# pavel-paulau/query

Hardware: AMD Instinct MI355X
Metric: rows/sec filter+group-by on 100M synthetic JSON docs; achieved HBM GB/s (higher is better)
Workload: dtype int64/f64 tagged scalars (u8 tag + 8 B payload), u32 dictionary codes; 1 GPU; config2: SELECT cat, SUM(price) FROM default WHERE price > 50 GROUP BY cat @ 100000000 rows, K_cat=1000, columns resident in HBM; rows_per_gpu=100000000, groups=1000, rows_selected=49401294, agg_mode=2, spec_kernel=1

## Files before the change

query_amd/build.py:

```python
from __future__ import annotations

import os
import shutil
import subprocess
import sys

HERE = os.path.dirname(os.path.abspath(__file__))
CSRC = os.path.join(HERE, "csrc")
LIB = os.path.join(HERE, "libn1k.so")
SOURCES = ["n1k_kernels.hip", "n1k_bins.hip", "n1k_jsondev.hip", "n1k_matchtable.hip", "n1k_order.hip", "n1k_rowdistinct.hip", "n1k_mathfn.hip", "n1k_arrfn.hip", "n1k_datefn.hip", "n1k_order.cpp", "n1k_rowdistinct.cpp", "n1k_matchtable.cpp", "n1k_like.cpp", "n1k_coll.cpp", "n1k_arrfn.cpp", "n1k_datefn.cpp", "n1k_in.cpp", "n1k_strfn.cpp", "n1k_jsonpush.cpp", "n1k_plan.cpp", "n1k_engine.cpp", "n1k_scan.cpp", "n1k_select.cpp", "n1k_partitioned.cpp", "n1k_distinct.cpp",
           "n1k_finish.cpp", "n1k_tail.cpp", "n1k_exchange.cpp", "n1k_jit.cpp", "n1k_json.cpp"]
HEADERS = ["n1k_types.h", "n1k_device.h", "n1k_tables.h", "n1k_fold.h", "n1k_scatter.h", "n1k_spec.h", "n1k_like.h", "n1k_coll.h", "n1k_arrfn.h", "n1k_datefn.h", "n1k_cond.h", "n1k_in.h", "n1k_strfn.h", "n1k_order.h", "n1k_rowdistinct.h", "n1k_jit.h", "n1k_kernels.h", "n1k_plan.h", os.path.join("..", "..", "include", "n1k.h")]
HOST_HEADERS = ["n1k_engine.h", "n1k_buf.h", "n1k_wire.h"]
ARCH = "gfx950"


def _hipcc() -> str:
    for c in (os.environ.get("HIPCC"), shutil.which("hipcc"), "/opt/rocm/bin/hipcc"):
        if c and os.path.exists(c):
            return c
    raise RuntimeError("hipcc not found")


OBJDIR = os.path.join(CSRC, "build")
FLAGS = ["--offload-arch=" + ARCH, "-O3", "-std=c++17", "-fPIC", "-munsafe-fp-atomics", "-Wall", "-Wno-unused-function"]


def _stale(target: str, deps) -> bool:
    if not os.path.exists(target):
        return True
    mt = os.path.getmtime(target)
    return any(os.path.getmtime(d) > mt for d in deps)


def source_hash() -> str:
    import hashlib
    h = hashlib.sha1()
    for f in sorted([x for x in SOURCES if x.endswith(".hip")] + [x for x in HEADERS if not x.startswith("..")]):
        with open(os.path.join(CSRC, f), "rb") as fh:
            h.update(f.encode() + b"\0" + fh.read())
    return h.hexdigest()[:16]


def needs_build() -> bool:
    return _stale(LIB, [os.path.join(CSRC, f) for f in SOURCES + HEADERS + HOST_HEADERS] + [os.path.abspath(__file__)])
# ... 33 lines not shown
```

query_amd/csrc/n1k_engine.h:

```cpp
#pragma once
#include <hip/hip_runtime.h>

#include <algorithm>
#include <atomic>
#include <chrono>
#include <cmath>
#include <cstdarg>
#include <cstdio>
#include <cstring>
#include <functional>
#include <numeric>
#include <string>
#include <condition_variable>
#include <mutex>
#include <thread>
#include <unordered_map>
#include <vector>

#include "../../include/n1k.h"
#include "n1k_buf.h"
#include "n1k_jit.h"
#include "n1k_json.h"
#include "n1k_kernels.h"
#include "n1k_arrfn.h"
// ... 148 lines not shown
    uint32_t jit = 1;
    uint64_t jit_min_rows = 4u << 20;
    uint32_t distinct_words = 1;
    uint32_t distinct_set_slots = 8192;
    uint32_t records = 1;
    uint32_t rec_slots = 0, rec_bins = 0, rec_slices = 0, rec_scan_per_cu = 0, rec_block = 0, rec_unroll = 0;
    uint64_t region_cap = 0;
    uint32_t dedupe_block = 1025;
    uint32_t json_device = 1;
    uint32_t json_device_left_pct = 12;
    uint64_t json_device_min_docs = 4096;
    uint32_t json_threads = 0;
    uint64_t partition_min_rows = 8u << 20, partition_probe_rows = 512u << 10, partition_min_groups = 4096;
    uint32_t partition_sticky = 1;
    int32_t partition_levels = -1;
    uint64_t topk_min_groups = 65536;
    int32_t distinct_levels = -1;
    uint64_t wide_values = 1u << 20;
    uint32_t slabs = 1;
    uint32_t block = 0, rows_per_lane = 4;
    uint32_t lds_bytes = 64 * 1024;
    uint32_t rep_row = 0;
    uint64_t rowdistinct_slots = 0;
    uint32_t rowdistinct_lds_slots = 0;
};

enum Counter : uint32_t {
    CTR_ROWS_SELECTED = 0,
    CTR_GROUPS = 1,
    CTR_OUT_COUNT = 2,
    CTR_FILTER_TOTAL = 3,
    CTR_REHASH_SCRATCH = 4,
    CTR_DISTINCT_REGION_WORDS = 5,
    CTR_TAIL_TICKET = 6,
    CTR_PAIR_LOG_CURSORS = 8,
    CTR_ERR_FLAGS = 12,
    CTR_WIDE_VALUES = 13,
    CTR_WORD_LOG_CURSORS = 16,
    CTR_OPTIMISTIC_OVERFLOW = 20,
    CTR_PART_RECORDS = 21,
    CTR_SINGLETONS = 22,
    CTR_EXACT_OVERFLOW = 24,
    CTR_SAVED_ROWS_SELECTED = 25,
    CTR_REGION_GROUPS = 26,
    CTR_PEER_STATUS = 27,
    CTR_ROWDISTINCT_COUNT = 28,
    CTR_ROWDISTINCT_REACHED = 29
};
static_assert(CTR_ERR_FLAGS + kPeerStatusFromErr == CTR_PEER_STATUS, "the verdict kernel writes the peer status this far behind the flags");
static_assert(CTR_ROWDISTINCT_REACHED < kCounters && CTR_ROWDISTINCT_REACHED == CTR_ROWDISTINCT_COUNT + 1, "every counter word lies inside the buffer (CTR_ROWDISTINCT_REACHED is the last)");
static_assert(CTR_ROWS_SELECTED == 0 && CTR_GROUPS == 1 && CTR_OUT_COUNT == 2 && CTR_TAIL_TICKET > CTR_DISTINCT_REGION_WORDS && CTR_TAIL_TICKET < CTR_PAIR_LOG_CURSORS,
              "the query's last kernels (finalize_small_kernel, fold_rows_kernel) write words [0], [1] and [2] by number");
static_assert(CTR_PAIR_LOG_CURSORS + kMaxDistinct <= CTR_ERR_FLAGS && CTR_WORD_LOG_CURSORS + kMaxDistinct <= CTR_OPTIMISTIC_OVERFLOW, "cursor words overlap their neighbours");

struct GroupTable {
    GlobalTable table{};
    DevBuf<uint64_t> keys, acc, rep;
    DevBuf<uint64_t> slabs;
    DevBuf<unsigned long long> block_sel;
    uint32_t* errp = nullptr;
    DevBuf<unsigned long long> counters;
    DevBuf<uint64_t> wide_int, wide_flt;
    uint64_t merged_bound = 0;
    struct PendingSlabs {
        bool clean_at_push = false;
        uint32_t grid = 0;
        FastArgs F{};
    } pending;
};
uint32_t intern(n1k_handle* h, const std::string& s);
uint32_t lookup_code(const n1k_handle* h, const char* s);
bool to_operand(n1k_handle* h, const Expr* e, Operand& o, PlanError& err);
bool compile_plan(n1k_handle* h, PlanError& err);
n1k_status ensure_device(n1k_handle* h);
n1k_status reset_handle(n1k_handle* h, bool clear_stop);
n1k_status ensure_rank(n1k_handle* h);
n1k_status fix_layout(n1k_handle* h, const n1k_batch* b);
n1k_status ensure_table(n1k_handle* h, uint64_t incoming_rows);
n1k_status ensure_table_groups(n1k_handle* h, uint64_t groups);
hipEvent_t get_event(n1k_handle* h);
n1k_status ensure_pinned_counters(n1k_handle* h);
void drain_events(n1k_handle* h);
n1k_status validate_batch(n1k_handle* h, const n1k_batch* b);
uint64_t batch_bytes_per_row(const n1k_handle* h);
void default_value(const AggDef& d, n1k_value& v, n1k_partial& p);
// ... 126 lines not shown
struct Distinct {
    DevBuf<uint64_t> log_key[kMaxDistinct], log_val[kMaxDistinct], regions, set_table;
    DevBuf<uint8_t> log_cls[kMaxDistinct];
    DevBuf<uint64_t> log_word[kMaxDistinct], part[2], seg[3], wtable;
    DevBuf<unsigned long long> hist, cursor, dcounts, word_hist;
    DevBuf<uint64_t> wregion[kMaxDistinct], woff, wgather;
    DevBuf<unsigned long long> wcursor;
    uint64_t wregion_cap = 0;
    bool wregion_used = false;
    uint32_t nw_key_bits = 0, nw_val_bits = 0;
    bool words[kMaxDistinct] = {false, false, false, false};
    uint32_t path = 0;
    uint64_t log_capacity = 0;
};
n1k_status distinct_grow_logs(n1k_handle* h, uint64_t nrows, ScanArgs& A);
n1k_status distinct_grow_regions(n1k_handle* h, const Program& P, uint64_t nrows, const ScanArgs& A, uint32_t dcache_slots, WordLogArgs& L);
n1k_status distinct_words_finish(n1k_handle* h, const AggSpec& ag, uint64_t nwords, bool hist_counted = true, const uint64_t* log = nullptr);
n1k_status distinct_regions_finish(n1k_handle* h, const AggSpec& ag, uint64_t nover, bool force_exact, bool* deferred);

struct TopK {
    DevBuf<uint64_t> images;
    DevBuf<uint32_t> cand;
    DevBuf<char> state, out2;
};
struct Results {
    std::vector<n1k_value> keys, aggs;
    std::vector<n1k_partial> parts;
    std::vector<uint64_t> rep;
    DevBuf<char> d_out;
    std::vector<char> out_host;
    std::vector<char> export_blob;
    bool out_count_dirty = true;
    PinBuf<char> pin_out;
    PinBuf<unsigned long long> pin_counters;
    PinBuf<char> pin_rows;
};

struct Tail {
    n1k_handle* project = nullptr;
    std::vector<int> project_cols;
    std::vector<Operand> project_ops;
    std::vector<n1k_value> r_proj;
    n1k_handle* having = nullptr;
    std::vector<int> having_cols;
    std::vector<uint32_t> having_codes;
};
n1k_status build_projection(n1k_handle* h);
n1k_status having_groups(n1k_handle* h, uint64_t& ng);
n1k_status project_groups(n1k_handle* h, uint64_t ng);
n1k_status order_groups(n1k_handle* h, uint64_t& ng);
n1k_status array_agg_groups(n1k_handle* h, uint64_t ng, const unsigned long long* counters);
bool slabs_to_rows(const n1k_handle* h, const FastArgs& F, uint32_t g, bool only_chunk, bool whole);
void publish_result(n1k_handle* h, uint64_t ng, bool partials, n1k_result* out);

}

using namespace n1k_eng;

struct n1k_handle {
    ParsedPlan plan;
    std::string last_error;
    std::atomic<int> stop_flag{0};
    Options opt;
    bool failure_global = false;
    bool device_clean = false, clear_on_finish = false;
    std::string jit_log;
// ... 74 lines not shown
```

query_amd/csrc/n1k_finish.cpp:

```cpp
#include "n1k_engine.h"

using namespace n1k;
using namespace n1k_eng;

static void mark_query_end(n1k_handle* h) {
    if (h->timing.q0_recorded && h->timing.ev_q1 && hipEventRecord(h->timing.ev_q1, h->stream) == hipSuccess) h->timing.q1_recorded = true;
}

struct OutLayout {
    size_t aggs, parts, rep, total;
    OutLayout(uint64_t groups = 0, size_t nk = 0, size_t na = 0)
        : aggs(groups * nk * sizeof(OutValue)), parts(aggs + groups * na * sizeof(OutValue)), rep(parts + groups * na * sizeof(OutPartial)), total(rep + groups * 8) {}
    OutValue* k(char* b) const { return (OutValue*)b; }
    OutValue* a(char* b) const { return (OutValue*)(b + aggs); }
    OutPartial* p(char* b) const { return (OutPartial*)(b + parts); }
    uint64_t* r(char* b) const { return (uint64_t*)(b + rep); }
};

struct Finish {
    unsigned long long counters[kCounters] = {0};
    uint32_t err_flags = 0;
    uint64_t ng = 0;
    uint64_t spec_groups = 0;
    char* d_rows = nullptr;
    char* rows = nullptr;
    OutLayout lay;
    bool sets_exact = false;
    bool sets_deferred = false, vetoed = false;
    std::chrono::steady_clock::time_point wait_end{};
};

enum : uint32_t { PIN_NCAND = kCounters, PIN_ERR_FLAGS, PIN_VETO };

static uint64_t speculative_groups(const n1k_handle* h) {
    const ParsedPlan& pl = h->plan;
    const bool topk_forced = pl.has_order && pl.limit >= 0 && !pl.has_having && h->opt.topk_min_groups < 4096;
    if (!pl.has_group || h->has_distinct || !h->groups.table.capacity || h->groups.table.capacity > (1u << 20) || topk_forced || h->part.pending.count)
        return 0;
    return std::min<uint64_t>(h->groups.table.capacity, 4096);
}

namespace n1k_eng {
bool slabs_to_rows(const n1k_handle* h, const FastArgs& F, uint32_t g, bool only_chunk, bool whole) {
    if (!h->clear_on_finish || !h->groups.pending.clean_at_push || !only_chunk || !whole || h->push_nrows_dev || h->push_nseg) return false;
    if (!F.slabs || F.hashed || g <= 1 || h->opt.merge_chunks != 0 || h->prog.wide_int || h->has_array_agg) return false;
    const uint64_t spec = speculative_groups(h), cap = h->groups.table.capacity;
    return spec && cap <= kFinalizeSmallMax && F.lds_slots <= std::min<uint64_t>(std::min<uint64_t>(cap, spec), h->opt.max_groups);
}
}

static n1k_status zero_out_count(n1k_handle* h) {
    if (h->res.out_count_dirty) HIP_TRY(h, hipMemsetAsync(h->groups.counters.p + CTR_OUT_COUNT, 0, sizeof(unsigned long long), h->stream));
    h->res.out_count_dirty = true;
    return N1K_OK;
}

static n1k_status read_counters(n1k_handle* h, Finish& F) {
    if (!h->device_ready) return h->timing.stats.rows_in == 0 ? ensure_device(h) : N1K_OK;
    HIP_TRY(h, hipSetDevice(h->device));
    ST_TRY(ensure_pinned_counters(h));
    GroupTable::PendingSlabs& ps = h->groups.pending;
    const bool fold = ps.grid && slabs_to_rows(h, ps.F, ps.grid, true, true);
    if (ps.grid && !fold) {
        HIP_TRY(h, launch_merge_slabs(h->prog, ps.F, h->groups.table, ps.grid, h->groups.counters.p + CTR_GROUPS, h->stream, h->opt.merge_chunks));
        ps.grid = 0;
    }
    F.spec_groups = speculative_groups(h);
    if (F.spec_groups) {
        F.lay = OutLayout(F.spec_groups, h->plan.keys.size(), h->plan.aggs.size());
        HIP_TRY(h, h->res.pin_out.ensure(F.lay.total + kCounters * sizeof(unsigned long long)));
        char* d = F.rows = h->res.pin_out.p;
        unsigned long long* host_counters = (unsigned long long*)(d + F.lay.total);
        if (fold) {
            HIP_TRY(h, launch_fold_rows(h->prog, ps.F, h->groups.table, ps.grid, F.lay.k(d), F.lay.a(d), F.lay.p(d), F.lay.r(d), h->groups.counters.p, CTR_TAIL_TICKET,
                                        host_counters, F.spec_groups, h->stream));
            ps.grid = 0;
            h->res.out_count_dirty = false;
            h->device_clean = true;
        } else if (h->groups.table.capacity <= kFinalizeSmallMax) {
            const bool clear = h->clear_on_finish && !h->prog.wide_int;
            HIP_TRY(h, launch_finalize_small(h->prog, h->groups.table, F.lay.k(d), F.lay.a(d), F.lay.p(d), F.lay.r(d), h->groups.counters.p,
                                             host_counters, F.spec_groups, h->groups.errp, clear, h->stream));
            h->res.out_count_dirty = !clear;
            h->device_clean = clear;
        } else {
            ST_TRY(zero_out_count(h));
            HIP_TRY(h, launch_finalize(h->prog, h->groups.table, F.lay.k(d), F.lay.a(d), F.lay.p(d), F.lay.r(d),
                                       h->groups.counters.p + CTR_OUT_COUNT, F.spec_groups, h->groups.errp, h->stream));
            HIP_TRY(h, launch_publish_counters(h->groups.counters.p, host_counters, kCounters, h->stream));
        }
        mark_query_end(h);
        const auto w0 = std::chrono::steady_clock::now();
        HIP_TRY(h, hipStreamSynchronize(h->stream));
        F.wait_end = std::chrono::steady_clock::now();
        h->timing.host_us[3] += std::chrono::duration<double, std::micro>(F.wait_end - w0).count();
        memcpy(F.counters, host_counters, sizeof F.counters);
        if (fold && F.counters[CTR_TAIL_TICKET]) {
            h->device_clean = false;
            F.counters[CTR_TAIL_TICKET] = 0;
        }
    } else {
        HIP_TRY(h, hipMemcpyAsync(h->res.pin_counters.p, h->groups.counters.p, sizeof F.counters, hipMemcpyDeviceToHost, h->stream));
        mark_query_end(h);
        HIP_TRY(h, hipStreamSynchronize(h->stream));
        memcpy(F.counters, h->res.pin_counters.p, sizeof F.counters);
    }
    F.err_flags = (uint32_t)F.counters[CTR_ERR_FLAGS];
    drain_events(h);
    return N1K_OK;
}

static n1k_status build_distinct_sets(n1k_handle* h, Finish& F) {
    h->distinct.path = 0;
    if (h->distinct.wregion_used) HIP_TRY(h, hipMemsetAsync(h->groups.counters.p + CTR_OPTIMISTIC_OVERFLOW, 0, 8, h->stream));
    for (size_t a = 0; a < h->plan.aggs.size(); a++) {
        const AggSpec& ag = h->prog.aggs[a];
        if (!ag.distinct || ag.kind == AGG_ARRAY) continue;
        const uint64_t npairs = std::min<uint64_t>(F.counters[CTR_PAIR_LOG_CURSORS + ag.log_index], h->distinct.log_capacity);
        const uint64_t nwords = h->distinct.words[ag.log_index] ? std::min<uint64_t>(F.counters[CTR_WORD_LOG_CURSORS + ag.log_index], h->distinct.log_capacity) : 0;
        DistinctArgs D{};
        D.log_key = h->distinct.log_key[ag.log_index].p;
        D.log_val = h->distinct.log_val[ag.log_index].p;
        D.log_cls = h->distinct.log_cls[ag.log_index].p;
        D.npairs = npairs;
        D.glob_off = ag.glob_off;
        D.kind = ag.kind;
        D.total_words = h->groups.counters.p + CTR_DISTINCT_REGION_WORDS;
        HIP_TRY(h, h->distinct.regions.ensure(h->groups.table.capacity * 6));
        D.regions = h->distinct.regions.p;
        HIP_TRY(h, hipMemsetAsync(D.total_words, 0, sizeof(unsigned long long), h->stream));
        HIP_TRY(h, launch_distinct_layout(h->prog, h->groups.table, D, h->stream));
        if (npairs) {
            unsigned long long words = 0;
// ... 70 lines not shown
    F.lay = OutLayout(ncand, nk, na);
    HIP_TRY(h, h->topk.out2.ensure(F.lay.total + 16));
    char* c = F.d_rows = h->topk.out2.p;
    if (tk.lean)
        HIP_TRY(h, launch_finalize_region(h->prog, h->part.emit.p, h->part.pending.cap, ncand, F.lay.k(c), F.lay.a(c), F.lay.p(c), F.lay.r(c),
                                          h->groups.errp, h->stream, h->topk.cand.p));
    else
        HIP_TRY(h, launch_topk_compact(h->topk.cand.p, ncand, nk, na, all.k(d), all.a(d), all.p(d), all.r(d), F.lay.k(c), F.lay.a(c), F.lay.p(c),
                                       F.lay.r(c), h->stream));
    h->timing.stats.topk_candidates = ncand;
    F.ng = ncand;
    return N1K_OK;
}

static n1k_status land_rows(n1k_handle* h, Finish& F) {
    const size_t bytes = F.lay.total;
    const bool pinned_rows = bytes <= (8u << 20);
    if (pinned_rows && h->res.pin_rows.n < bytes) HIP_TRY(h, h->res.pin_rows.ensure(std::max<size_t>(bytes, 64u << 10)));
    if (!pinned_rows) h->res.out_host.resize(bytes);
    F.rows = pinned_rows ? h->res.pin_rows.p : h->res.out_host.data();
    unsigned long long* const pin = h->res.pin_counters.p;
    HIP_TRY(h, hipMemcpyAsync(F.rows, F.d_rows, bytes, hipMemcpyDeviceToHost, h->stream));
    HIP_TRY(h, hipMemcpyAsync(pin + PIN_ERR_FLAGS, h->groups.errp, 4, hipMemcpyDeviceToHost, h->stream));
    if (F.sets_deferred) HIP_TRY(h, hipMemcpyAsync(pin + PIN_VETO, h->groups.counters.p + CTR_OPTIMISTIC_OVERFLOW, 8, hipMemcpyDeviceToHost, h->stream));
    mark_query_end(h);
    HIP_TRY(h, hipStreamSynchronize(h->stream));
    memcpy(&F.err_flags, pin + PIN_ERR_FLAGS, 4);
    F.vetoed = F.sets_deferred && pin[PIN_VETO] != 0;
    return N1K_OK;
}

static void unpack_rows(n1k_handle* h, const Finish& F) {
    const size_t nk = h->plan.keys.size(), na = h->plan.aggs.size(), ng = F.ng;
    h->res.keys.assign((const n1k_value*)F.lay.k(F.rows), (const n1k_value*)F.lay.k(F.rows) + ng * nk);
    h->res.aggs.assign((const n1k_value*)F.lay.a(F.rows), (const n1k_value*)F.lay.a(F.rows) + ng * na);
    h->res.rep.assign(F.lay.r(F.rows), F.lay.r(F.rows) + ng);
    const OutPartial* parts = F.lay.p(F.rows);
    h->res.parts.resize(ng * na);
    for (size_t i = 0; i < ng * na; i++) {
        n1k_partial& p = h->res.parts[i];
        memset(&p, 0, sizeof p);
        p.count = parts[i].count;
        p.isum = parts[i].isum;
        p.fsum = parts[i].fsum;
        p.int_exact = parts[i].flags & 1u;
        p.has_float = (parts[i].flags >> 1) & 1u;
        p.extreme.tag = (uint8_t)parts[i].ext_tag;
        p.extreme.v.code = parts[i].ext_payload;
        p.distinct = parts[i].distinct;
    }
}

static n1k_status flags_status(n1k_handle* h, const Finish& F) {
    if (F.err_flags & kErrFromVerdict) {
        h->failure_global = true;
        if (F.err_flags & ERR_PEER_FAILED) {
            const int ps = (int)(F.counters[CTR_PEER_STATUS] & 0xFF);
            return fail(h, ps > 0 && ps <= N1K_REGION_FULL ? (n1k_status)ps : N1K_DEVICE_ERROR,
                        "a rank failed before the exchange (its status: %d); the step is void on every rank", ps);
        }
        if (F.err_flags & ERR_EXCHANGE_WIDE)
            return fail(h, N1K_UNSUPPORTED, "a sender's group keys hold float / wide integer values: use the row exchange");
        if (F.err_flags & ERR_EXCHANGE_OVERFLOW)
            return fail(h, N1K_REGION_FULL, "a sender's region overflowed: raise the region capacity (on every rank)");
        if (F.err_flags & ERR_PEER_UNPACKABLE)
            return fail(h, N1K_UNSUPPORTED_DATA, "a sender met a group key value that does not fit the packed key (option wide_values, or a key layout too narrow)");
        return fail(h, N1K_UNSUPPORTED_DATA, "a sender met a value outside the device subset (ordering of arrays/objects)");
    }
    if (F.err_flags & ERR_TABLE_FULL)
        return fail(h, N1K_OOM, "group table capacity exceeded: raise the max_groups option (now %llu)",
                    (unsigned long long)h->opt.max_groups);
    if (F.err_flags & ERR_UNPACKABLE_KEY)
        return fail(h, N1K_UNSUPPORTED_DATA,
                    "a group key value does not fit the packed key: more than %llu distinct float / wide integer key "
                    "values (option wide_values), or a key layout too narrow for them",
                    (unsigned long long)((1ull << h->prog.wide_bits) / 2));
    if (F.err_flags & ERR_UNSUPPORTED_VALUE)
        return fail(h, N1K_UNSUPPORTED_DATA, "a value outside the device subset was met (ordering of arrays/objects)");
    return N1K_OK;
}

static n1k_status host_tail(n1k_handle* h, uint64_t ng, n1k_result* out) {
// ... 72 lines not shown
```

query_amd/csrc/n1k_kernels.h:

```cpp
#pragma once
#include <hip/hip_runtime.h>
#include <vector>
#include "n1k_types.h"
#include "n1k_cond.h"

namespace n1k {

constexpr int kFilterStreamTile = 8192;
constexpr uint32_t kFinalizeSmallMax = 8192;

struct OutValue {
    uint64_t tag;
    uint64_t payload;
};

struct OutPartial {
    int64_t count;
    int64_t isum;
    double fsum;
    uint32_t flags;
    uint32_t ext_tag;
    uint64_t ext_payload;
    int64_t distinct;
};

struct SynthArgs {
    uint64_t seed, first_row, nrows, total_rows;
    uint32_t k_cat, pad;
    const double* cat_cdf;
    uint32_t* cat_codes;
    uint8_t* price_tags;
    uint64_t* price_payload;
    uint8_t* user_tags;
    uint64_t* user_payload;
    uint8_t* region_tags;
    uint64_t* region_payload;
};
// ... 51 lines not shown
                                 uint64_t limit = 0, bool unique_keys = false);
hipError_t launch_arith(const ArithArgs& A, hipStream_t st);
hipError_t launch_mathfn(const ArithArgs& A, hipStream_t st);
hipError_t launch_datefn(const ArithArgs& A, hipStream_t st);
hipError_t launch_cond(const Program& P, const CondArgs& C, hipStream_t st);
hipError_t launch_publish_counters(const unsigned long long* src, unsigned long long* dst, uint32_t n, hipStream_t st);
hipError_t launch_partition(const Program& P, const PartArgs& A, uint32_t grid, hipStream_t st);
struct HeaderList { unsigned long long* h[kMaxParts]; };
hipError_t launch_exchange_verdict(const HeaderList& H, uint32_t nregions, uint32_t* err_flags, hipStream_t st);
hipError_t launch_stamp_verdict(unsigned long long* headers, uint32_t nregions, uint64_t stride_words, const uint32_t* err_flags,
                                uint32_t host_status, hipStream_t st);
hipError_t launch_dense_to_segments(unsigned long long* headers, uint32_t nregions, uint64_t stride_words, uint64_t sub_rows, hipStream_t st,
                                    const uint32_t* dest_cap = nullptr);
struct SpecEntry {
    const char* name;
    SpecSig sig;
    hipError_t (*launch)(const Program& P, const FastArgs& F, const GlobalTable& G, unsigned long long* ngroups,
                         uint32_t grid, uint32_t block, bool wide, const WordLogArgs& L, hipStream_t st);
    hipError_t (*launch_records)(const Program& P, const FastArgs& F, uint32_t grid, bool wide, const WordLogArgs& L, hipStream_t st);
};
size_t spec_records_lds_bytes();
hipError_t launch_radix_scatter16(const RadixArgs& A, uint32_t wpr, uint32_t bins_per_region, hipStream_t st);
hipError_t launch_radix_scatter_words(const RadixArgs& A, uint32_t wpr, uint32_t bins_per_region, hipStream_t st);
size_t agg_bins16_lds_bytes(const Program& P, uint32_t slots);
hipError_t launch_agg_bins16(const Program& P, const BinAggArgs& A, uint32_t grid, uint32_t block, uint32_t per_thread, hipStream_t st,
                             bool specialise = true);
const std::vector<SpecEntry>& spec_registry();
hipError_t launch_finalize(const Program& P, const GlobalTable& G, OutValue* out_keys, OutValue* out_aggs,
                           OutPartial* out_parts, uint64_t* out_rep, unsigned long long* out_count, uint64_t max_out,
                           uint32_t* err_flags, hipStream_t st);
hipError_t launch_finalize_small(const Program& P, const GlobalTable& G, OutValue* out_keys, OutValue* out_aggs, OutPartial* out_parts,
                                 uint64_t* out_rep, unsigned long long* counters, unsigned long long* host_counters, uint64_t max_out,
                                 uint32_t* err_flags, bool clear, hipStream_t st);
hipError_t launch_fold_rows(const Program& P, const FastArgs& F, const GlobalTable& G, uint32_t nslabs, OutValue* out_keys, OutValue* out_aggs,
                            OutPartial* out_parts, uint64_t* out_rep, unsigned long long* counters, uint32_t ticket_word,
                            unsigned long long* host_counters, uint64_t max_out, hipStream_t st);
hipError_t launch_filter_stream(const Program& P, uint64_t nrows, uint64_t row_base, uint64_t* out_rows, unsigned long long* tile_state,
                                unsigned long long* tile_counter, unsigned long long* total, uint32_t* err_flags, uint32_t grid,
                                hipStream_t st, bool fast = false);
hipError_t launch_filter_stream(const Program& P, uint64_t nrows, uint32_t* out_rows, unsigned long long* tile_state,
                                unsigned long long* tile_counter, unsigned long long* total, uint32_t* err_flags, uint32_t grid,
                                hipStream_t st, bool fast);
constexpr uint32_t kGatherMaxCols = 16;
struct GatherCol {
    uint32_t kind, pad;
    const uint8_t* src_tags;
    const uint64_t* src_payload;
    const uint32_t* src_codes;
    uint8_t* dst_tags;
    uint64_t* dst_payload;
    uint32_t* dst_codes;
};
struct GatherArgs {
    const uint32_t* rows;
    uint64_t n;
    uint32_t ncols, pad;
    GatherCol cols[kGatherMaxCols];
};
hipError_t launch_gather_rows(const GatherArgs& A, hipStream_t st);
constexpr uint32_t kJsonMaxSteps = 4;
struct JsonDevPath {
    uint32_t nsteps;
    uint32_t name_off[kJsonMaxSteps], name_len[kJsonMaxSteps];
};
struct JsonDevArgs {
    const uint8_t* bytes;
    const uint64_t* offsets;
    uint64_t base, ndocs;
    uint32_t npaths, tab_bits;
// ... 20 lines not shown
```

query_amd/csrc/n1k_kernels.hip:

```cpp
#include <hip/hip_runtime.h>
#include "n1k_device.h"
#include "n1k_tables.h"
#include "n1k_fold.h"
#include "n1k_scatter.h"
#include "n1k_kernels.h"
#include <algorithm>
#include <vector>

namespace n1k {


template <int R>
N1K_DEV void load_operand(const Program& P, const Operand& o, const uint64_t (&row)[R], const bool (&valid)[R],
                          uint32_t (&tag)[R], uint64_t (&pay)[R]) {
    if (o.is_const) {
#pragma unroll
        for (int j = 0; j < R; j++) {
            tag[j] = o.ctag;
            pay[j] = o.cpayload;
        }
        return;
    }
    const DevCol& c = P.cols[o.col];
    if (c.kind == COLK_DICT32) {
// ... 1800 lines not shown
        if (clear) {
            G.keys[s] = kEmptyKey;
            if (G.rep_row) G.rep_row[s] = ~0ull;
            glob_row_init(P, g);
        }
    }
    __syncthreads();
    if (tid == 0) counters[2] = next;
    __syncthreads();
    if (tid < kCounters) {
        host_counters[tid] = __hip_atomic_load(&counters[tid], __ATOMIC_RELAXED, __HIP_MEMORY_SCOPE_AGENT);
        if (clear) counters[tid] = 0;
    }
}

hipError_t launch_finalize_small(const Program& P, const GlobalTable& G, OutValue* out_keys, OutValue* out_aggs, OutPartial* out_parts,
                                 uint64_t* out_rep, unsigned long long* counters, unsigned long long* host_counters, uint64_t max_out,
                                 uint32_t* err_flags, bool clear, hipStream_t st) {
    if (G.capacity > kFinalizeSmallMax) return hipErrorInvalidValue;
    hipLaunchKernelGGL(finalize_small_kernel, dim3(1), dim3(1024), 0, st, P, G, out_keys, out_aggs, out_parts, out_rep, counters,
                       host_counters, max_out, err_flags, clear ? 1u : 0u);
    return hipGetLastError();
}

#ifndef N1K_FOLD_SLOTS
#define N1K_FOLD_SLOTS 16
#endif
#ifndef N1K_FOLD_CHUNK
#define N1K_FOLD_CHUNK 6
#endif
constexpr uint32_t kFoldSlots = N1K_FOLD_SLOTS, kFoldChunk = N1K_FOLD_CHUNK;
constexpr uint32_t kFoldStage = kFoldMaxWords + 1;
static_assert(kFoldSlots == 4 || kFoldSlots == 8 || kFoldSlots == 16 || kFoldSlots == 32, "slots of a workgroup share a wave");

template <uint32_t KIND, uint32_t SLOTS, bool KEY>
N1K_DEV void fold_rows_agg(const uint64_t* key0, const uint64_t* l, uint32_t S, size_t slab_words, uint32_t nslabs, uint32_t bl,
                           uint64_t* acc, uint64_t& touched) {
    constexpr uint32_t LANES = 1024 / SLOTS, NW = fold_slab_words(KIND), CH = NW <= 3 || kFoldChunk < 4 ? kFoldChunk : 4;
    fold_init(KIND, acc);
    for (uint32_t b0 = 0; b0 < nslabs; b0 += LANES * CH) {
        uint64_t x[CH][kFoldMaxWords], k[CH];
#pragma unroll
        for (uint32_t c = 0; c < CH; c++) {
            const uint32_t b = b0 + c * LANES + bl;
            const size_t at = (size_t)(b < nslabs ? b : 0u) * slab_words;
            k[c] = KEY ? key0[at] : kEmptyKey;
#pragma unroll
            for (uint32_t i = 0; i < NW; i++) x[c][i] = l[at + i * (size_t)S];
        }
#pragma unroll
        for (uint32_t c = 0; c < CH; c++) {
            const bool valid = b0 + c * LANES + bl < nslabs;
#pragma unroll
            for (uint32_t i = 0; i < NW; i++) x[c][i] = valid ? x[c][i] : fold_slab_identity(KIND, i);
            touched |= valid ? (k[c] ^ kEmptyKey) : 0ull;
            fold_slab(KIND, acc, x[c]);
        }
    }
    for (uint32_t off = SLOTS; off < 64; off <<= 1) {
        uint64_t other[kFoldMaxWords];
#pragma unroll
        for (uint32_t i = 0; i < fold_acc_words(KIND); i++) other[i] = (uint64_t)__shfl_xor((unsigned long long)acc[i], (int)off, 64);
        fold_join(KIND, acc, other);
        if (KEY) touched |= (uint64_t)__shfl_xor((unsigned long long)touched, (int)off, 64);
    }
}

template <uint32_t SLOTS, bool KEY>
N1K_DEV void fold_rows_kind(uint32_t kind, const uint64_t* key0, const uint64_t* l, uint32_t S, size_t slab_words, uint32_t nslabs,
                            uint32_t bl, uint64_t* acc, uint64_t& touched) {
    switch (kind) {
        case AGG_COUNT:
        case AGG_COUNTN: fold_rows_agg<AGG_COUNT, SLOTS, KEY>(key0, l, S, slab_words, nslabs, bl, acc, touched); break;
        case AGG_SUM: fold_rows_agg<AGG_SUM, SLOTS, KEY>(key0, l, S, slab_words, nslabs, bl, acc, touched); break;
        case AGG_AVG: fold_rows_agg<AGG_AVG, SLOTS, KEY>(key0, l, S, slab_words, nslabs, bl, acc, touched); break;
        case AGG_MIN: fold_rows_agg<AGG_MIN, SLOTS, KEY>(key0, l, S, slab_words, nslabs, bl, acc, touched); break;
        default: fold_rows_agg<AGG_MAX, SLOTS, KEY>(key0, l, S, slab_words, nslabs, bl, acc, touched); break;
    }
}

template <uint32_t SLOTS>
__global__ __launch_bounds__(1024) void fold_rows_kernel(const Program P, const FastArgs F, const GlobalTable G, uint32_t nslabs,
                                                        OutValue* out_keys, OutValue* out_aggs, OutPartial* out_parts,
                                                        uint64_t* out_rep, unsigned long long* counters, uint32_t ticket_word,
                                                        unsigned long long* host_counters, uint64_t max_out) {
    __shared__ uint64_t stage[16][SLOTS][kFoldStage];
    __shared__ uint64_t accs[SLOTS][kMaxAggs][kFoldMaxWords];
    __shared__ uint64_t rows[SLOTS][kMaxAggs * kFoldMaxWords];
    __shared__ uint64_t touched_s[SLOTS];
    const uint32_t tid = threadIdx.x, lane = tid & 63, wave = tid >> 6, sx = tid % SLOTS, bl = tid / SLOTS;
    const uint32_t S = F.lds_slots;
    const uint32_t s = blockIdx.x * SLOTS + sx;
    const size_t slab_words = (size_t)P.lds_words * S;
    const uint64_t* key0 = F.slabs + (s < S ? s : S - 1);
    unsigned long long in_table = 0, sel = 0;
    if (wave == 0) {
        in_table = __hip_atomic_load(&counters[1], __ATOMIC_RELAXED, __HIP_MEMORY_SCOPE_AGENT);
        const uint32_t per = (nslabs + gridDim.x - 1) / gridDim.x, lo = blockIdx.x * per, hi = lo + per < nslabs ? lo + per : nslabs;
        for (uint32_t b = lo + lane; b < hi; b += 64) sel += F.block_selected[b];
    }
    for (uint32_t a = 0; a < P.naggs; a++) {
        const AggSpec& ag = P.aggs[a];
        const uint64_t* l = key0 + (size_t)ag.lds_off * S;
        uint64_t acc[kFoldMaxWords], touched = 0;
        const bool first = a == 0;
        if (first) fold_rows_kind<SLOTS, true>(ag.kind, key0, l, S, slab_words, nslabs, bl, acc, touched);
        else fold_rows_kind<SLOTS, false>(ag.kind, key0, l, S, slab_words, nslabs, bl, acc, touched);
        const uint32_t na = fold_acc_words(ag.kind);
        if (lane < SLOTS) {
#pragma unroll
            for (uint32_t i = 0; i < kFoldMaxWords; i++)
                if (i < na) stage[wave][sx][i] = acc[i];
            if (first) stage[wave][sx][kFoldMaxWords] = touched;
        }
        __syncthreads();
        if (tid < SLOTS * kFoldStage && (bl < na || (first && bl == kFoldMaxWords))) {
            const uint32_t op = bl == kFoldMaxWords ? (uint32_t)FOLD_OR : fold_word_op(ag.kind, bl);
            uint64_t v = stage[0][sx][bl];
            for (uint32_t w = 1; w < 16; w++) v = fold_word(op, v, stage[w][sx][bl]);
            if (bl == kFoldMaxWords) touched_s[sx] = v;
            else accs[sx][a][bl] = v;
        }
        __syncthreads();
    }
    if (wave != 0) return;
    for (int off = 32; off > 0; off >>= 1) sel += __shfl_xor(sel, off, 64);
    if (lane == 0 && sel) atomicAdd(&counters[0], sel);
    {
        const bool used = tid < SLOTS && s < S && touched_s[tid % SLOTS] != 0;
        const unsigned long long m = __ballot(used);
        unsigned long long first = 0;
        if (tid == 0 && m) first = atomicAdd(&counters[2], (unsigned long long)__popcll(m));
        first = __shfl(first, 0, 64);
        const unsigned long long idx = first + (uint32_t)__popcll(m & ((1ull << lane) - 1ull));
        if (used && idx < max_out) {
            uint64_t* g = rows[tid % SLOTS];
            const uint64_t key = fast_slot_key(F, s);
            if (in_table) {
                const uint64_t mask = G.capacity - 1;
                uint64_t at = mix64(key) & mask;
                for (uint64_t probe = 0; probe < G.capacity; probe++, at = (at + 1) & mask) {
                    const uint64_t cur = G.keys[at];
                    if (cur == kEmptyKey) break;
                    if (cur != key) continue;
                    for (uint32_t a = 0; a < P.naggs; a++)
                        fold_join(P.aggs[a].kind, accs[tid % SLOTS][a], &G.acc[at * P.glob_words + P.aggs[a].glob_off]);
                    break;
                }
            }
            for (uint32_t a = 0; a < P.naggs; a++) fold_row(P.aggs[a].kind, accs[tid % SLOTS][a], g + P.aggs[a].glob_off);
            for (uint32_t k = 0; k < P.nkeys; k++) {
                const KeySpec& ks = P.keys[k];
                uint64_t field = ks.bits >= 64 ? key : ((key >> ks.shift) & ((1ull << ks.bits) - 1ull));
                uint32_t tag;
                uint64_t p;
                unpack_key_field(P, ks.mode, field, tag, p);
                put_value(&out_keys[idx * P.nkeys + k], tag, p);
            }
            for (uint32_t a = 0; a < P.naggs; a++)
                finalize_agg(P, P.aggs[a], g, &out_aggs[idx * P.naggs + a], &out_parts[idx * P.naggs + a], F.err_flags);
            if (out_rep) out_rep[idx] = P.emit_packed_key ? key : ~0ull;
        }
    }
    uint32_t last = 0;
    __threadfence();
    if (lane == 0) last = atomicAdd(&counters[ticket_word], 1ull) == (unsigned long long)gridDim.x - 1ull ? 1u : 0u;
    if (!__shfl(last, 0, 64)) return;
    __threadfence();
    unsigned long long v = __hip_atomic_load(&counters[lane % kCounters], __ATOMIC_RELAXED, __HIP_MEMORY_SCOPE_AGENT);
    const unsigned long long nrows_out = __shfl(v, 2, 64);
    in_table = __shfl(v, 1, 64);
    if (lane == 1 || lane == 2) v = nrows_out;
    if (lane == ticket_word) v = in_table;
    if (lane < kCounters) {
        host_counters[lane] = v;
        counters[lane] = 0;
    }
}

hipError_t launch_fold_rows(const Program& P, const FastArgs& F, const GlobalTable& G, uint32_t nslabs, OutValue* out_keys,
                            OutValue* out_aggs, OutPartial* out_parts, uint64_t* out_rep, unsigned long long* counters,
                            uint32_t ticket_word, unsigned long long* host_counters, uint64_t max_out, hipStream_t st) {
    if (!G.capacity || (G.capacity & (G.capacity - 1)) || !F.slabs || !F.block_selected || !nslabs || !F.lds_slots || F.hashed) return hipErrorInvalidValue;
    if (ticket_word < 3 || ticket_word >= kCounters || P.naggs == 0) return hipErrorInvalidValue;
    for (uint32_t a = 0; a < P.naggs; a++)
        if (P.aggs[a].distinct || P.aggs[a].kind > AGG_MAX) return hipErrorInvalidValue;
    hipLaunchKernelGGL(fold_rows_kernel<kFoldSlots>, dim3((F.lds_slots + kFoldSlots - 1) / kFoldSlots), dim3(1024), 0, st, P, F, G,
                       nslabs, out_keys, out_aggs, out_parts, out_rep, counters, ticket_word, host_counters, max_out);
    return hipGetLastError();
}

N1K_DEV uint64_t order_image(const Program& P, uint64_t tag, uint64_t p, bool desc);
__global__ void finalize_region_kernel(const Program P, const uint64_t* region, uint64_t cap, uint64_t count, OutValue* out_keys,
                                       OutValue* out_aggs, OutPartial* out_parts, uint64_t* out_rep, uint32_t* err_flags,
                                       const uint32_t* cand, OutValue* ord, uint32_t ord_is_key, uint32_t ord_index, uint64_t* images,
                                       uint32_t desc) {
    const uint64_t j = (uint64_t)blockIdx.x * blockDim.x + threadIdx.x;
    if (j >= count) return;
    const uint64_t i = cand ? (uint64_t)cand[j] : j;
    const uint64_t key = region[2 + i];
    const uint64_t* g = region + 2 + cap + i * P.glob_words;
    if (ord || images) {
        OutValue v, term;
        OutPartial part;
        term.tag = T_MISSING;
        term.payload = 0;
        for (uint32_t a = 0; a < P.naggs; a++) {
            finalize_agg(P, P.aggs[a], g, &v, &part, err_flags);
            if (!ord_is_key && a == ord_index) term = v;
        }
        if (ord_is_key) {
            const KeySpec& ks = P.keys[ord_index];
            uint64_t field = ks.bits >= 64 ? key : ((key >> ks.shift) & ((1ull << ks.bits) - 1ull));
            uint32_t tag;
            uint64_t p;
            unpack_key_field(P, ks.mode, field, tag, p);
            put_value(&term, tag, p);
        }
        if (images) images[i] = order_image(P, term.tag, term.payload, desc != 0);
        else ord[i] = term;
        return;
// ... 1278 lines not shown
```

Measured before the change: 347.0 billion rows/s.

## Replace fold_rows global atomics and last-block ticket with per-workgroup records decoded on host

```diff
diff --git a/query_amd/build.py b/query_amd/build.py
--- a/query_amd/build.py
+++ b/query_amd/build.py
@@ -10,7 +10,7 @@
 LIB = os.path.join(HERE, "libn1k.so")
 SOURCES = ["n1k_kernels.hip", "n1k_bins.hip", "n1k_jsondev.hip", "n1k_matchtable.hip", "n1k_order.hip", "n1k_rowdistinct.hip", "n1k_mathfn.hip", "n1k_arrfn.hip", "n1k_datefn.hip", "n1k_order.cpp", "n1k_rowdistinct.cpp", "n1k_matchtable.cpp", "n1k_like.cpp", "n1k_coll.cpp", "n1k_arrfn.cpp", "n1k_datefn.cpp", "n1k_in.cpp", "n1k_strfn.cpp", "n1k_jsonpush.cpp", "n1k_plan.cpp", "n1k_engine.cpp", "n1k_scan.cpp", "n1k_select.cpp", "n1k_partitioned.cpp", "n1k_distinct.cpp",
            "n1k_finish.cpp", "n1k_tail.cpp", "n1k_exchange.cpp", "n1k_jit.cpp", "n1k_json.cpp"]
-HEADERS = ["n1k_types.h", "n1k_device.h", "n1k_tables.h", "n1k_fold.h", "n1k_scatter.h", "n1k_spec.h", "n1k_like.h", "n1k_coll.h", "n1k_arrfn.h", "n1k_datefn.h", "n1k_cond.h", "n1k_in.h", "n1k_strfn.h", "n1k_order.h", "n1k_rowdistinct.h", "n1k_jit.h", "n1k_kernels.h", "n1k_plan.h", os.path.join("..", "..", "include", "n1k.h")]
+HEADERS = ["n1k_types.h", "n1k_device.h", "n1k_tables.h", "n1k_fold.h", "n1k_rows.h", "n1k_scatter.h", "n1k_spec.h", "n1k_like.h", "n1k_coll.h", "n1k_arrfn.h", "n1k_datefn.h", "n1k_cond.h", "n1k_in.h", "n1k_strfn.h", "n1k_order.h", "n1k_rowdistinct.h", "n1k_jit.h", "n1k_kernels.h", "n1k_plan.h", os.path.join("..", "..", "include", "n1k.h")]
 HOST_HEADERS = ["n1k_engine.h", "n1k_buf.h", "n1k_wire.h"]
 ARCH = "gfx950"
 
diff --git a/query_amd/csrc/n1k_engine.h b/query_amd/csrc/n1k_engine.h
--- a/query_amd/csrc/n1k_engine.h
+++ b/query_amd/csrc/n1k_engine.h
@@ -204,7 +204,6 @@
     CTR_FILTER_TOTAL = 3,
     CTR_REHASH_SCRATCH = 4,
     CTR_DISTINCT_REGION_WORDS = 5,
-    CTR_TAIL_TICKET = 6,
     CTR_PAIR_LOG_CURSORS = 8,
     CTR_ERR_FLAGS = 12,
     CTR_WIDE_VALUES = 13,
@@ -221,8 +220,7 @@
 };
 static_assert(CTR_ERR_FLAGS + kPeerStatusFromErr == CTR_PEER_STATUS, "the verdict kernel writes the peer status this far behind the flags");
 static_assert(CTR_ROWDISTINCT_REACHED < kCounters && CTR_ROWDISTINCT_REACHED == CTR_ROWDISTINCT_COUNT + 1, "every counter word lies inside the buffer (CTR_ROWDISTINCT_REACHED is the last)");
-static_assert(CTR_ROWS_SELECTED == 0 && CTR_GROUPS == 1 && CTR_OUT_COUNT == 2 && CTR_TAIL_TICKET > CTR_DISTINCT_REGION_WORDS && CTR_TAIL_TICKET < CTR_PAIR_LOG_CURSORS,
-              "the query's last kernels (finalize_small_kernel, fold_rows_kernel) write words [0], [1] and [2] by number");
+static_assert(CTR_ROWS_SELECTED == 0 && CTR_GROUPS == 1 && CTR_OUT_COUNT == 2, "the query's last kernel (finalize_small_kernel) writes word [2] by number");
 static_assert(CTR_PAIR_LOG_CURSORS + kMaxDistinct <= CTR_ERR_FLAGS && CTR_WORD_LOG_CURSORS + kMaxDistinct <= CTR_OPTIMISTIC_OVERFLOW, "cursor words overlap their neighbours");
 
 struct GroupTable {
@@ -415,6 +413,7 @@
     std::vector<char> export_blob;
     bool out_count_dirty = true;
     PinBuf<char> pin_out;
+    std::vector<uint32_t> fold_slots;
     PinBuf<unsigned long long> pin_counters;
     PinBuf<char> pin_rows;
 };
diff --git a/query_amd/csrc/n1k_finish.cpp b/query_amd/csrc/n1k_finish.cpp
--- a/query_amd/csrc/n1k_finish.cpp
+++ b/query_amd/csrc/n1k_finish.cpp
@@ -25,6 +25,7 @@
     char* d_rows = nullptr;
     char* rows = nullptr;
     OutLayout lay;
+    const uint32_t* slots = nullptr;
     bool sets_exact = false;
     bool sets_deferred = false, vetoed = false;
     std::chrono::steady_clock::time_point wait_end{};
@@ -68,15 +69,19 @@
     F.spec_groups = speculative_groups(h);
     if (F.spec_groups) {
         F.lay = OutLayout(F.spec_groups, h->plan.keys.size(), h->plan.aggs.size());
-        HIP_TRY(h, h->res.pin_out.ensure(F.lay.total + kCounters * sizeof(unsigned long long)));
+        const size_t behind = (F.lay.total + 15) & ~(size_t)15;
+        const uint32_t fold_slots = fold ? fold_rows_slots() : 1u;
+        HIP_TRY(h, h->res.pin_out.ensure(behind + std::max(kCounters * sizeof(unsigned long long), fold ? fold_records_bytes(fold_record_count(ps.F.lds_slots, fold_slots)) : 0)));
         char* d = F.rows = h->res.pin_out.p;
         unsigned long long* host_counters = (unsigned long long*)(d + F.lay.total);
+        FoldHead* const fold_head = (FoldHead*)(d + behind);
+        FoldRecord* const fold_recs = (FoldRecord*)(fold_head + 1);
+        const uint32_t fold_S = ps.F.lds_slots;
         if (fold) {
-            HIP_TRY(h, launch_fold_rows(h->prog, ps.F, h->groups.table, ps.grid, F.lay.k(d), F.lay.a(d), F.lay.p(d), F.lay.r(d), h->groups.counters.p, CTR_TAIL_TICKET,
-                                        host_counters, F.spec_groups, h->stream));
+            HIP_TRY(h, launch_fold_rows(h->prog, ps.F, h->groups.table, ps.grid, F.lay.k(d), F.lay.a(d), F.lay.p(d), F.lay.r(d), h->groups.counters.p + CTR_GROUPS,
+                                        fold_head, fold_recs, F.spec_groups, h->stream));
             ps.grid = 0;
             h->res.out_count_dirty = false;
-            h->device_clean = true;
         } else if (h->groups.table.capacity <= kFinalizeSmallMax) {
             const bool clear = h->clear_on_finish && !h->prog.wide_int;
             HIP_TRY(h, launch_finalize_small(h->prog, h->groups.table, F.lay.k(d), F.lay.a(d), F.lay.p(d), F.lay.r(d), h->groups.counters.p,
@@ -94,11 +99,16 @@
         HIP_TRY(h, hipStreamSynchronize(h->stream));
         F.wait_end = std::chrono::steady_clock::now();
         h->timing.host_us[3] += std::chrono::duration<double, std::micro>(F.wait_end - w0).count();
-        memcpy(F.counters, host_counters, sizeof F.counters);
-        if (fold && F.counters[CTR_TAIL_TICKET]) {
-            h->device_clean = false;
-            F.counters[CTR_TAIL_TICKET] = 0;
-        }
+        if (fold) {
+            if (h->res.fold_slots.size() < fold_S) h->res.fold_slots.resize(fold_S);
+            F.slots = h->res.fold_slots.data();
+            const FoldSummary sum = fold_records_decode(*fold_head, fold_recs, fold_S, fold_slots, h->res.fold_slots.data());
+            F.counters[CTR_ROWS_SELECTED] = sum.selected;
+            F.counters[CTR_GROUPS] = F.counters[CTR_OUT_COUNT] = sum.groups;
+            F.counters[CTR_ERR_FLAGS] = sum.err_flags;
+            h->device_clean = sum.in_table == 0 && sum.err_flags == 0;
+        } else
+            memcpy(F.counters, host_counters, sizeof F.counters);
     } else {
         HIP_TRY(h, hipMemcpyAsync(h->res.pin_counters.p, h->groups.counters.p, sizeof F.counters, hipMemcpyDeviceToHost, h->stream));
         mark_query_end(h);
@@ -235,22 +245,34 @@
 
 static void unpack_rows(n1k_handle* h, const Finish& F) {
     const size_t nk = h->plan.keys.size(), na = h->plan.aggs.size(), ng = F.ng;
-    h->res.keys.assign((const n1k_value*)F.lay.k(F.rows), (const n1k_value*)F.lay.k(F.rows) + ng * nk);
-    h->res.aggs.assign((const n1k_value*)F.lay.a(F.rows), (const n1k_value*)F.lay.a(F.rows) + ng * na);
-    h->res.rep.assign(F.lay.r(F.rows), F.lay.r(F.rows) + ng);
-    const OutPartial* parts = F.lay.p(F.rows);
+    const OutPartial* const all_parts = F.lay.p(F.rows);
+    if (F.slots) {
+        h->res.keys.resize(ng * nk);
+        h->res.aggs.resize(ng * na);
+        h->res.rep.resize(ng);
+        fold_rows_gather(h->res.keys.data(), F.lay.k(F.rows), nk * sizeof(n1k_value), F.slots, ng);
+        fold_rows_gather(h->res.aggs.data(), F.lay.a(F.rows), na * sizeof(n1k_value), F.slots, ng);
+        fold_rows_gather(h->res.rep.data(), F.lay.r(F.rows), sizeof(uint64_t), F.slots, ng);
+    } else {
+        h->res.keys.assign((const n1k_value*)F.lay.k(F.rows), (const n1k_value*)F.lay.k(F.rows) + ng * nk);
+        h->res.aggs.assign((const n1k_value*)F.lay.a(F.rows), (const n1k_value*)F.lay.a(F.rows) + ng * na);
+        h->res.rep.assign(F.lay.r(F.rows), F.lay.r(F.rows) + ng);
+    }
     h->res.parts.resize(ng * na);
-    for (size_t i = 0; i < ng * na; i++) {
-        n1k_partial& p = h->res.parts[i];
-        memset(&p, 0, sizeof p);
-        p.count = parts[i].count;
-        p.isum = parts[i].isum;
-        p.fsum = parts[i].fsum;
-        p.int_exact = parts[i].flags & 1u;
-        p.has_float = (parts[i].flags >> 1) & 1u;
-        p.extreme.tag = (uint8_t)parts[i].ext_tag;
-        p.extreme.v.code = parts[i].ext_payload;
-        p.distinct = parts[i].distinct;
+    for (size_t r = 0; r < ng; r++) {
+        const OutPartial* parts = all_parts + (F.slots ? F.slots[r] : r) * na;
+        for (size_t a = 0; a < na; a++) {
+            n1k_partial& p = h->res.parts[r * na + a];
+            memset(&p, 0, sizeof p);
+            p.count = parts[a].count;
+            p.isum = parts[a].isum;
+            p.fsum = parts[a].fsum;
+            p.int_exact = parts[a].flags & 1u;
+            p.has_float = (parts[a].flags >> 1) & 1u;
+            p.extreme.tag = (uint8_t)parts[a].ext_tag;
+            p.extreme.v.code = parts[a].ext_payload;
+            p.distinct = parts[a].distinct;
+        }
     }
 }
 
diff --git a/query_amd/csrc/n1k_kernels.h b/query_amd/csrc/n1k_kernels.h
--- a/query_amd/csrc/n1k_kernels.h
+++ b/query_amd/csrc/n1k_kernels.h
@@ -3,6 +3,7 @@
 #include <vector>
 #include "n1k_types.h"
 #include "n1k_cond.h"
+#include "n1k_rows.h"
 
 namespace n1k {
 
@@ -120,9 +121,10 @@
 hipError_t launch_finalize_small(const Program& P, const GlobalTable& G, OutValue* out_keys, OutValue* out_aggs, OutPartial* out_parts,
                                  uint64_t* out_rep, unsigned long long* counters, unsigned long long* host_counters, uint64_t max_out,
                                  uint32_t* err_flags, bool clear, hipStream_t st);
+uint32_t fold_rows_slots();
 hipError_t launch_fold_rows(const Program& P, const FastArgs& F, const GlobalTable& G, uint32_t nslabs, OutValue* out_keys, OutValue* out_aggs,
-                            OutPartial* out_parts, uint64_t* out_rep, unsigned long long* counters, uint32_t ticket_word,
-                            unsigned long long* host_counters, uint64_t max_out, hipStream_t st);
+                            OutPartial* out_parts, uint64_t* out_rep, const unsigned long long* ngroups, FoldHead* head,
+                            FoldRecord* records, uint64_t max_out, hipStream_t st);
 hipError_t launch_filter_stream(const Program& P, uint64_t nrows, uint64_t row_base, uint64_t* out_rows, unsigned long long* tile_state,
                                 unsigned long long* tile_counter, unsigned long long* total, uint32_t* err_flags, uint32_t grid,
                                 hipStream_t st, bool fast = false);
diff --git a/query_amd/csrc/n1k_kernels.hip b/query_amd/csrc/n1k_kernels.hip
--- a/query_amd/csrc/n1k_kernels.hip
+++ b/query_amd/csrc/n1k_kernels.hip
@@ -1856,6 +1856,7 @@
 constexpr uint32_t kFoldSlots = N1K_FOLD_SLOTS, kFoldChunk = N1K_FOLD_CHUNK;
 constexpr uint32_t kFoldStage = kFoldMaxWords + 1;
 static_assert(kFoldSlots == 4 || kFoldSlots == 8 || kFoldSlots == 16 || kFoldSlots == 32, "slots of a workgroup share a wave");
+static_assert(kFoldSlots <= kFoldRecordSlotsMax, "a FoldRecord has a bit per slot");
 
 template <uint32_t KIND, uint32_t SLOTS, bool KEY>
 N1K_DEV void fold_rows_agg(const uint64_t* key0, const uint64_t* l, uint32_t S, size_t slab_words, uint32_t nslabs, uint32_t bl,
@@ -1906,20 +1907,24 @@
 template <uint32_t SLOTS>
 __global__ __launch_bounds__(1024) void fold_rows_kernel(const Program P, const FastArgs F, const GlobalTable G, uint32_t nslabs,
                                                         OutValue* out_keys, OutValue* out_aggs, OutPartial* out_parts,
-                                                        uint64_t* out_rep, unsigned long long* counters, uint32_t ticket_word,
-                                                        unsigned long long* host_counters, uint64_t max_out) {
+                                                        uint64_t* out_rep, const unsigned long long* ngroups, FoldHead* head,
+                                                        FoldRecord* records) {
     __shared__ uint64_t stage[16][SLOTS][kFoldStage];
     __shared__ uint64_t accs[SLOTS][kMaxAggs][kFoldMaxWords];
     __shared__ uint64_t rows[SLOTS][kMaxAggs * kFoldMaxWords];
     __shared__ uint64_t touched_s[SLOTS];
+    __shared__ uint32_t raised;
+    if (threadIdx.x == 0) raised = 0;
     const uint32_t tid = threadIdx.x, lane = tid & 63, wave = tid >> 6, sx = tid % SLOTS, bl = tid / SLOTS;
     const uint32_t S = F.lds_slots;
     const uint32_t s = blockIdx.x * SLOTS + sx;
     const size_t slab_words = (size_t)P.lds_words * S;
     const uint64_t* key0 = F.slabs + (s < S ? s : S - 1);
     unsigned long long in_table = 0, sel = 0;
+    uint32_t scan_flags = 0;
     if (wave == 0) {
-        in_table = __hip_atomic_load(&counters[1], __ATOMIC_RELAXED, __HIP_MEMORY_SCOPE_AGENT);
+        in_table = __hip_atomic_load(ngroups, __ATOMIC_RELAXED, __HIP_MEMORY_SCOPE_AGENT);
+        if (blockIdx.x == 0) scan_flags = __hip_atomic_load(F.err_flags, __ATOMIC_RELAXED, __HIP_MEMORY_SCOPE_AGENT);
         const uint32_t per = (nslabs + gridDim.x - 1) / gridDim.x, lo = blockIdx.x * per, hi = lo + per < nslabs ? lo + per : nslabs;
         for (uint32_t b = lo + lane; b < hi; b += 64) sel += F.block_selected[b];
     }
@@ -1949,68 +1954,63 @@
     }
     if (wave != 0) return;
     for (int off = 32; off > 0; off >>= 1) sel += __shfl_xor(sel, off, 64);
-    if (lane == 0 && sel) atomicAdd(&counters[0], sel);
-    {
-        const bool used = tid < SLOTS && s < S && touched_s[tid % SLOTS] != 0;
-        const unsigned long long m = __ballot(used);
-        unsigned long long first = 0;
-        if (tid == 0 && m) first = atomicAdd(&counters[2], (unsigned long long)__popcll(m));
-        first = __shfl(first, 0, 64);
-        const unsigned long long idx = first + (uint32_t)__popcll(m & ((1ull << lane) - 1ull));
-        if (used && idx < max_out) {
-            uint64_t* g = rows[tid % SLOTS];
-            const uint64_t key = fast_slot_key(F, s);
-            if (in_table) {
-                const uint64_t mask = G.capacity - 1;
-                uint64_t at = mix64(key) & mask;
-                for (uint64_t probe = 0; probe < G.capacity; probe++, at = (at + 1) & mask) {
-                    const uint64_t cur = G.keys[at];
-                    if (cur == kEmptyKey) break;
-                    if (cur != key) continue;
-                    for (uint32_t a = 0; a < P.naggs; a++)
-                        fold_join(P.aggs[a].kind, accs[tid % SLOTS][a], &G.acc[at * P.glob_words + P.aggs[a].glob_off]);
-                    break;
-                }
-            }
-            for (uint32_t a = 0; a < P.naggs; a++) fold_row(P.aggs[a].kind, accs[tid % SLOTS][a], g + P.aggs[a].glob_off);
-            for (uint32_t k = 0; k < P.nkeys; k++) {
-                const KeySpec& ks = P.keys[k];
-                uint64_t field = ks.bits >= 64 ? key : ((key >> ks.shift) & ((1ull << ks.bits) - 1ull));
-                uint32_t tag;
-                uint64_t p;
-                unpack_key_field(P, ks.mode, field, tag, p);
-                put_value(&out_keys[idx * P.nkeys + k], tag, p);
-            }
-            for (uint32_t a = 0; a < P.naggs; a++)
-                finalize_agg(P, P.aggs[a], g, &out_aggs[idx * P.naggs + a], &out_parts[idx * P.naggs + a], F.err_flags);
-            if (out_rep) out_rep[idx] = P.emit_packed_key ? key : ~0ull;
-        }
-    }
-    uint32_t last = 0;
-    __threadfence();
-    if (lane == 0) last = atomicAdd(&counters[ticket_word], 1ull) == (unsigned long long)gridDim.x - 1ull ? 1u : 0u;
-    if (!__shfl(last, 0, 64)) return;
-    __threadfence();
-    unsigned long long v = __hip_atomic_load(&counters[lane % kCounters], __ATOMIC_RELAXED, __HIP_MEMORY_SCOPE_AGENT);
-    const unsigned long long nrows_out = __shfl(v, 2, 64);
-    in_table = __shfl(v, 1, 64);
-    if (lane == 1 || lane == 2) v = nrows_out;
-    if (lane == ticket_word) v = in_table;
-    if (lane < kCounters) {
-        host_counters[lane] = v;
-        counters[lane] = 0;
-    }
-}
+    const bool used = tid < SLOTS && s < S && touched_s[tid % SLOTS] != 0;
+    const unsigned long long m = __ballot(used);
+    if (used) {
+        uint64_t* g = rows[tid % SLOTS];
+        const uint64_t key = fast_slot_key(F, s);
+        if (in_table) {
+            const uint64_t mask = G.capacity - 1;
+            uint64_t at = mix64(key) & mask;
+            for (uint64_t probe = 0; probe < G.capacity; probe++, at = (at + 1) & mask) {
+                const uint64_t cur = G.keys[at];
+                if (cur == kEmptyKey) break;
+                if (cur != key) continue;
+                for (uint32_t a = 0; a < P.naggs; a++)
+                    fold_join(P.aggs[a].kind, accs[tid % SLOTS][a], &G.acc[at * P.glob_words + P.aggs[a].glob_off]);
+                break;
+            }
+        }
+        for (uint32_t a = 0; a < P.naggs; a++) fold_row(P.aggs[a].kind, accs[tid % SLOTS][a], g + P.aggs[a].glob_off);
+        const size_t idx = s;
+        for (uint32_t k = 0; k < P.nkeys; k++) {
+            const KeySpec& ks = P.keys[k];
+            uint64_t field = ks.bits >= 64 ? key : ((key >> ks.shift) & ((1ull << ks.bits) - 1ull));
+            uint32_t tag;
+            uint64_t p;
+            unpack_key_field(P, ks.mode, field, tag, p);
+            put_value(&out_keys[idx * P.nkeys + k], tag, p);
+        }
+        for (uint32_t a = 0; a < P.naggs; a++)
+            finalize_agg(P, P.aggs[a], g, &out_aggs[idx * P.naggs + a], &out_parts[idx * P.naggs + a], &raised);
+        if (out_rep) out_rep[idx] = P.emit_packed_key ? key : ~0ull;
+    }
+    __builtin_amdgcn_fence(__ATOMIC_ACQ_REL, "workgroup");
+    if (lane != 0) return;
+    FoldRecord rec;
+    rec.selected = sel;
+    rec.used = (uint32_t)m;
+    rec.flags = __hip_atomic_load(&raised, __ATOMIC_RELAXED, __HIP_MEMORY_SCOPE_WORKGROUP);
+    records[blockIdx.x] = rec;
+    if (blockIdx.x == 0) {
+        FoldHead hd;
+        hd.in_table = in_table;
+        hd.err_flags = scan_flags;
+        *head = hd;
+    }
+}
+
+uint32_t fold_rows_slots() { return kFoldSlots; }
 
 hipError_t launch_fold_rows(const Program& P, const FastArgs& F, const GlobalTable& G, uint32_t nslabs, OutValue* out_keys,
-                            OutValue* out_aggs, OutPartial* out_parts, uint64_t* out_rep, unsigned long long* counters,
-                            uint32_t ticket_word, unsigned long long* host_counters, uint64_t max_out, hipStream_t st) {
+                            OutValue* out_aggs, OutPartial* out_parts, uint64_t* out_rep, const unsigned long long* ngroups,
+                            FoldHead* head, FoldRecord* records, uint64_t max_out, hipStream_t st) {
     if (!G.capacity || (G.capacity & (G.capacity - 1)) || !F.slabs || !F.block_selected || !nslabs || !F.lds_slots || F.hashed) return hipErrorInvalidValue;
-    if (ticket_word < 3 || ticket_word >= kCounters || P.naggs == 0) return hipErrorInvalidValue;
+    if (F.lds_slots > max_out || !ngroups || !F.err_flags || !head || !records || P.naggs == 0) return hipErrorInvalidValue;
     for (uint32_t a = 0; a < P.naggs; a++)
         if (P.aggs[a].distinct || P.aggs[a].kind > AGG_MAX) return hipErrorInvalidValue;
-    hipLaunchKernelGGL(fold_rows_kernel<kFoldSlots>, dim3((F.lds_slots + kFoldSlots - 1) / kFoldSlots), dim3(1024), 0, st, P, F, G,
-                       nslabs, out_keys, out_aggs, out_parts, out_rep, counters, ticket_word, host_counters, max_out);
+    hipLaunchKernelGGL(fold_rows_kernel<kFoldSlots>, dim3(fold_record_count(F.lds_slots, kFoldSlots)), dim3(1024), 0, st, P, F, G,
+                       nslabs, out_keys, out_aggs, out_parts, out_rep, ngroups, head, records);
     return hipGetLastError();
 }
 
diff --git a/query_amd/csrc/n1k_rows.h b/query_amd/csrc/n1k_rows.h
--- /dev/null
+++ b/query_amd/csrc/n1k_rows.h
@@ -0,0 +1,57 @@
+#pragma once
+#include <cstddef>
+#include <cstdint>
+#include <cstring>
+
+namespace n1k {
+
+constexpr uint32_t kFoldRecordSlotsMax = 32;
+
+struct alignas(16) FoldRecord {
+    uint64_t selected;
+    uint32_t used;
+    uint32_t flags;
+};
+
+struct alignas(16) FoldHead {
+    uint64_t in_table;
+    uint64_t err_flags;
+};
+
+static_assert(sizeof(FoldRecord) == 16 && sizeof(FoldHead) == 16, "one 16-byte store each");
+
+constexpr uint32_t fold_record_count(uint32_t S, uint32_t per_wg) { return (S + per_wg - 1) / per_wg; }
+constexpr size_t fold_records_bytes(uint32_t nrec) { return sizeof(FoldHead) + (size_t)nrec * sizeof(FoldRecord); }
+
+struct FoldSummary {
+    uint64_t groups = 0, selected = 0, in_table = 0;
+    uint32_t err_flags = 0;
+};
+
+inline FoldSummary fold_records_decode(const FoldHead& head, const FoldRecord* recs, uint32_t S, uint32_t per_wg, uint32_t* slots) {
+    FoldSummary r;
+    r.in_table = head.in_table;
+    r.err_flags = (uint32_t)head.err_flags;
+    const uint32_t nrec = fold_record_count(S, per_wg);
+    for (uint32_t w = 0; w < nrec; w++) {
+        r.selected += recs[w].selected;
+        r.err_flags |= recs[w].flags;
+        const uint32_t base = w * per_wg, n = S - base < per_wg ? S - base : per_wg;
+        uint32_t m = n >= 32 ? recs[w].used : (recs[w].used & ((1u << n) - 1u));
+        for (; m; m &= m - 1) slots[r.groups++] = base + (uint32_t)__builtin_ctz(m);
+    }
+    return r;
+}
+
+inline void fold_rows_gather(void* dst, const void* src, size_t elem, const uint32_t* slots, size_t n) {
+    char* d = (char*)dst;
+    const char* s = (const char*)src;
+    for (size_t i = 0; i < n;) {
+        size_t j = i + 1;
+        while (j < n && slots[j] == slots[j - 1] + 1) j++;
+        memcpy(d + i * elem, s + (size_t)slots[i] * elem, (j - i) * elem);
+        i = j;
+    }
+}
+
+}
```

Result: no change. 349.5 billion rows/s (median of 6 runs) (+0.7%).
